# ThomasBrouwer/BNMTF

Hardware: AMD Instinct MI355X
Metric: Gibbs iterations/sec (BNMF, I=J=8192, K=64) (higher is better)
Workload: dtype f32

## Files before the change

bnmtf_amd/csrc/api.hip:

```cpp
#include <algorithm>
#include <atomic>
#include <chrono>
#include <cmath>
#include <cstdarg>
#include <cstdio>
#include <cstring>
#include <mutex>
#include <exception>
#include <new>
#include <system_error>
#include <thread>
#include <tuple>
#include <vector>

#include "model.h"
#include "comm.h"
#include "many.h"
#include "device_rng.h"

namespace bnmtf {

static thread_local char g_err[1024] = "";
void set_error(const char* fmt, ...) {
  va_list ap;
// ... 399 lines not shown
static bool build_handover(bnmtf_model* h, Dir& W, Dir& Rd) {
  if (!W.f_row_blk || !Rd.f_row_blk || W.f_npairs == 0 || Rd.f_npairs == 0) return false;
  const int nbW = (W.f_npairs + W.ho_ppb - 1) / W.ho_ppb, nbR = (Rd.f_npairs + Rd.ho_ppb - 1) / Rd.ho_ppb;
  if (nbR > 8192) return false;
  const size_t rowsW = W.f_slots, rowsR = Rd.f_slots;
  DevBuf<uint32_t> inv, dst_slot, dst_rank, count, sbase, stotal, rbase, rdata, rsize, limits;
  if (inv.alloc(std::max<size_t>(Rd.nslots, 1)) || dst_slot.alloc(std::max<size_t>(rowsW, 1) * 64) || dst_rank.alloc(std::max<size_t>(rowsW, 1) * 64) ||
      count.alloc((size_t)nbW * nbR) || sbase.alloc((size_t)nbW * nbR) || stotal.alloc(nbW) || rbase.alloc((size_t)nbW * nbR) || rdata.alloc(nbR) ||
      rsize.alloc(nbR) || limits.alloc(4, true)) return false;
  uint16_t *t_out = nullptr, *t_in = nullptr;
  if (dalloc(&t_out, ((rowsW + 1) / 2) * 128, true) || dalloc(&t_in, ((rowsR + 1) / 2) * 128, true)) return false;
  W.ho_out = reinterpret_cast<uint32_t*>(t_out); Rd.ho_in = reinterpret_cast<uint32_t*>(t_in);
  if (dalloc(&W.ho_pk, (size_t)nbW * nbR * 3, false) || dalloc(&Rd.ho_region_ofs, (size_t)nbR + 1, false)) return false;
  HandoverArgs a;
  a.w_off = W.f_off; a.w_pB = W.f_pair_base; a.w_pE = W.f_pair_E; a.w_umap = W.f_unit_map; a.w_npairs = W.f_npairs; a.w_ppb = W.ho_ppb; a.w_nb = nbW; a.w_inner = (uint32_t)Rd.nglob;
  a.r_off = Rd.f_off; a.r_pB = Rd.f_pair_base; a.r_pE = Rd.f_pair_E; a.r_umap = Rd.f_unit_map; a.r_npairs = Rd.f_npairs; a.r_ppb = Rd.ho_ppb; a.r_nb = nbR; a.r_inner = (uint32_t)W.nglob;
  a.r_row_blk = Rd.f_row_blk; a.r_ptr = Rd.slot_ptr; a.r_idx = Rd.idx;
  a.inv = inv.p; a.dst_slot = dst_slot.p; a.dst_rank = dst_rank.p; a.count = count.p;
  a.sbase = sbase.p; a.stotal = stotal.p; a.rbase = rbase.p; a.rdata = rdata.p; a.rsize = rsize.p;
  a.rofs = Rd.ho_region_ofs; a.t_out = t_out; a.t_in = t_in; a.pk = W.ho_pk; a.limits = limits.p;
  launch_handover_build(a, h->stream);
  uint32_t lim[4];
  if (hipMemcpyAsync(lim, limits.p, sizeof(lim), hipMemcpyDeviceToHost, h->stream) != hipSuccess || hipStreamSynchronize(h->stream) != hipSuccess) return false;
  const uint32_t lds_w = (W.ho_ppb == 8 ? 80u : 160u) * 1024u / 4u - (uint32_t)(W.KP * W.KP) - 256u;
  const uint32_t lds_r = (Rd.ho_ppb == 8 ? 80u : 160u) * 1024u / 4u - (uint32_t)(W.KP * W.KP) - 256u;
  if (lim[2] != 0 || lim[0] + 256u + 32u > lds_w || lim[0] + 32u > 65536u || lim[1] > lds_r || lim[1] > 65536u) return false;
  W.ho_lds_floats = std::max(W.ho_lds_floats, (int)lim[0] + 256 + 32);
  Rd.ho_lds_floats = std::max(Rd.ho_lds_floats, (int)lim[1]);
  if (dalloc(&Rd.ho_region, (size_t)lim[3] + 256) != BNMTF_OK) return false;
  Rd.ho_blocks = nbR;
  return true;
}

static int alloc_factor(Dir& d, int other_inner_pad) {
  d.xrows = std::max(d.nglob + 1, other_inner_pad);
  d.ldT = round_up(round_up(d.nglob, 32) + 32, 256);
  CHK(dalloc(&d.X, (size_t)d.xrows * d.KP));
  CHK(dalloc(&d.XT, (size_t)d.KP * d.ldT));
  CHK(dalloc(&d.XT2, (size_t)d.KP * d.ldT));
  const int nb = post_blocks(d.nglob);
  CHK(dalloc(&d.Cpart, (size_t)nb * d.KP * d.KP));
  CHK(dalloc(&d.spart, (size_t)nb * d.KP));
  CHK(dalloc(&d.s2part, (size_t)nb * d.KP));
  return BNMTF_OK;
}

static void free_dir(Dir& d) {
  dfree(d.big); dfree(d.slabs); dfree(d.lambda); dfree(d.slot_ptr); dfree(d.idx); dfree(d.q);
  dfree(d.X); dfree(d.XT); dfree(d.C64); dfree(d.C32);
  if (!d.gram_packed) { dfree(d.colsum); dfree(d.colsum2); }
  if (d.ev_sweep) (void)hipEventDestroy(d.ev_sweep);
  if (d.ev_gram) (void)hipEventDestroy(d.ev_gram);
  if (d.ev_gathered) (void)hipEventDestroy(d.ev_gathered);
  if (d.ev_gram_all) (void)hipEventDestroy(d.ev_gram_all);
  dfree(d.XT2); dfree(d.Cpart); dfree(d.spart); dfree(d.s2part); dfree(d.f_unit_map); dfree(d.f_pair_E);
  dfree(d.f_pair_base); dfree(d.f_off); dfree(d.f_off16); dfree(d.stats); dfree(d.f_gen_units);
  dfree(d.u_unit_map); dfree(d.u_pair_E); dfree(d.u_pair_base); dfree(d.u_off16);
  dfree(d.vb_stats);
  dfree(d.ho_in); dfree(d.ho_out); dfree(d.ho_pk); dfree(d.ho_region_ofs); dfree(d.ho_region); dfree(d.f_row_blk);
  dfree(d.mu); dfree(d.tauq); dfree(d.var); dfree(d.S2); dfree(d.S2T); dfree(d.XS); dfree(d.vb_asq); dfree(d.vb_vsq); dfree(d.mbits); dfree(d.XB); dfree(d.mslabs); dfree(d.xb_umax); dfree(d.xb_cexp); dfree(d.xb_mpart); dfree(d.numer); dfree(d.taup);
}

struct ScopedKernelTimer {
  bnmtf_model* h; int id; hipEvent_t a = nullptr, b = nullptr;
  bool on;
  ScopedKernelTimer(bnmtf_model* h_, int id_) : h(h_), id(id_), on(((h_->profiling >> id_) & 1u) && h_->iteration % h_->profile_stride == 0) {
    if (!on) return;
    auto get = [&]() {
      hipEvent_t e;
      if (!h->event_pool.empty()) { e = h->event_pool.back(); h->event_pool.pop_back(); }
      else (void)hipEventCreate(&e);
      return e;
    };
    a = get(); b = get();
    (void)hipEventRecord(a, h->stream);
  }
  ~ScopedKernelTimer() {
    if (!on) return;
    (void)hipEventRecord(b, h->stream);
    h->pending_events.push_back({id, {a, b}});
  }
};
static void drain_events(bnmtf_model* h) {
  for (auto& pe : h->pending_events) {
    float ms = 0.f;
    if (hipEventElapsedTime(&ms, pe.second.first, pe.second.second) == hipSuccess) {
      h->kernel_ms[pe.first] += ms;
      h->kernel_launches[pe.first] += 1;
    }
    h->event_pool.push_back(pe.second.first);
    h->event_pool.push_back(pe.second.second);
  }
  h->pending_events.clear();
}

struct HandoverScope {
  bnmtf_model* h;
  explicit HandoverScope(bnmtf_model* h_) : h(h_) {
    h->ho_active = h->ho_enabled && !h->comm && h->use_fast && !h->block_mode;
    if (!h->ho_active || !h->ho_regions_current) h->rows.ho_filled = h->cols.ho_filled = false;
    h->ho_regions_current = false;
  }
  void commit() { h->ho_regions_current = h->ho_active && h->rows.ho_filled; }
  ~HandoverScope() { h->ho_active = false; }
};
static void enqueue_gemm(bnmtf_model* h, Dir& d, const Dir& other, int kid, int part = 0);
static void enqueue_gemm(bnmtf_model* h, Dir& d, const Dir& other, int kid, int part) {
  GemmArgs g;
  g.big = d.big; g.ld = d.n_pad; g.X = other.X; g.slabs = d.slabs;
  g.n_pad = d.n_pad; g.split = d.split; g.inner_per_wave = d.ipw; g.tw = d.gemm_tw;
  const int rows_per_slice = 4 * d.ipw;
  const int s0 = (other.n0 + rows_per_slice - 1) / rows_per_slice, s1 = std::min(d.split, (other.n0 + other.n) / rows_per_slice);
  const bool have_local = h->comm && s1 > s0;
  if (part == 1) {
    if (!have_local) return;
    ScopedKernelTimer t(h, kid);
    g.split0 = s0; g.nsplit = s1 - s0;
    launch_gemm(g, d.KP, h->stream);
    return;
  }
  ScopedKernelTimer t(h, kid);
  if (part == 2 && have_local) {
    if (s0 > 0) { g.split0 = 0; g.nsplit = s0; launch_gemm(g, d.KP, h->stream); }
    if (s1 < d.split) { g.split0 = s1; g.nsplit = d.split - s1; launch_gemm(g, d.KP, h->stream); }
    return;
  }
  launch_gemm(g, d.KP, h->stream);
}
static bool vb_chip_ok(const Dir& d, const Dir& o) {
  if (!(d.mbits && o.XB && d.mslabs && d.nch == 1 && sweep_fast_supported(d.KP, d.pw))) return false;
  if (d.vb_path != 0) return d.vb_path == 1;
  return d.KP == 64 && d.use_wide;
}
static void enqueue_post(bnmtf_model* h, Dir& d, bool vb = false) {
  PostArgs g;
  memset(&g, 0, sizeof(g));
  g.X = d.X; g.rows = d.nglob; g.KP = d.KP; g.XT = d.XT; g.ldT = d.ldT; g.XT2 = d.XT2; g.ld2 = d.ldT;
  g.Cpart = d.Cpart; g.spart = d.spart; g.C64 = d.C64; g.C32 = d.C32; g.colsum = d.colsum;
  if (vb) { g.S2 = d.S2; g.S2T = d.S2T; g.s2part = d.s2part; g.colsum2 = d.colsum2; g.XS = d.XS; }
  if (vb && vb_chip_ok(h->rows, h->cols) && vb_chip_ok(h->cols, h->rows)) {
    g.XS = nullptr;
    g.mpart = d.xb_mpart; g.umax = d.xb_umax;
    d.xb_umax_posted = d.xb_mpart != nullptr;
  } else d.xb_umax_posted = false;
  g.snap = d.snap_dst; g.snapW = d.W; d.snap_dst = nullptr;
  launch_post(g, h->stream);
}
static int exchange_factor(bnmtf_model* h, Dir& d, Dir* next = nullptr, int next_kid = 0) {
  if (!h->comm) { enqueue_post(h, d); return BNMTF_OK; }
  const char* xe = getenv("BNMTF_EXCHANGE");
  if (xe && !strcmp(xe, "serial")) {
    PostArgs g;
    memset(&g, 0, sizeof(g));
    g.X = d.X; g.rows = d.nglob; g.KP = d.KP; g.XT = d.XT; g.ldT = d.ldT; g.XT2 = d.XT2; g.ld2 = d.ldT;
    g.Cpart = d.Cpart; g.spart = d.spart; g.C64 = d.C64; g.C32 = d.C32; g.colsum = d.colsum;
    launch_post_gram_rows(g, d.n0, d.n0 + d.n, h->stream);
    CHK(comm_allgather_factor(h->comm, d.X, d.KP, d.nglob, h->world, h->stream));
    CHK(comm_allreduce_sum(h->comm, d.C64, 64 * 64 + 64, h->stream));
    launch_gram_cast(d.C64, d.C32, d.KP * d.KP, h->stream);
    g.snap = d.snap_dst; g.snapW = d.W; d.snap_dst = nullptr;
    launch_post_layout(g, h->stream);
    d.gram_pending = false;
    return BNMTF_OK;
  }
  if (!h->xchg_stream) HIPCHK(hipStreamCreateWithFlags(&h->xchg_stream, hipStreamNonBlocking));
  for (hipEvent_t* e : {&d.ev_sweep, &d.ev_gram, &d.ev_gathered, &d.ev_gram_all})
    if (!*e) HIPCHK(hipEventCreateWithFlags(e, hipEventDisableTiming));
  PostArgs g;
  memset(&g, 0, sizeof(g));
  g.X = d.X; g.rows = d.nglob; g.KP = d.KP; g.XT = d.XT; g.ldT = d.ldT; g.XT2 = d.XT2; g.ld2 = d.ldT;
  g.Cpart = d.Cpart; g.spart = d.spart; g.C64 = d.C64; g.C32 = d.C32; g.colsum = d.colsum;
  HIPCHK(hipEventRecord(d.ev_sweep, h->stream));
  launch_post_gram_rows(g, d.n0, d.n0 + d.n, h->stream);
  HIPCHK(hipEventRecord(d.ev_gram, h->stream));
  if (next) enqueue_gemm(h, *next, d, next_kid, 1);
  HIPCHK(hipStreamWaitEvent(h->xchg_stream, d.ev_sweep, 0));
  CHK(comm_allgather_factor(h->comm, d.X, d.KP, d.nglob, h->world, h->xchg_stream));
  HIPCHK(hipEventRecord(d.ev_gathered, h->xchg_stream));
  HIPCHK(hipStreamWaitEvent(h->xchg_stream, d.ev_gram, 0));
  CHK(comm_allreduce_sum(h->comm, d.C64, 64 * 64 + 64, h->xchg_stream));
  launch_gram_cast(d.C64, d.C32, d.KP * d.KP, h->xchg_stream);
  HIPCHK(hipEventRecord(d.ev_gram_all, h->xchg_stream));
// ... 33 lines not shown
    s2.acc = nullptr;
    if (h->ho_active) { d.ho_filled = false; }
    launch_sweep_unit(s2, f, h->stream);
    h->last_sweep_fast = true;
    return;
  }
  if (h->use_fast && d.fast_ok && s.cond_k < 0 && s.mode != kSweepVB && (d.nch == 2 || sweep_fast_supported(d.KP, d.pw))) {
    FastArgs f;
    f.unit_map = d.f_unit_map; f.pair_E = d.f_pair_E; f.pair_base = d.f_pair_base; f.off = d.f_off;
    f.npairs = d.f_npairs; f.mz = d.mz; f.pw = d.nch == 2 ? d.pw_chunk : d.pw; f.nw = d.f_nw;
    f.nch = d.nch; f.mh = d.mh; f.pw1 = d.pw1; f.twin = d.use_twin ? 1 : 0;
    f.XoT = other.XT; f.ldT_o = other.ldT; f.XoT2 = other.XT2; f.ld2_o = other.ldT; f.Xo = other.X; f.Xo_rows = other.nglob;
    f.stats = want_stats ? d.stats : nullptr;
    SweepArgs s2 = s;
    s2.acc = nullptr;
    f.off16 = d.pair_ok ? d.f_off16 : nullptr;
    set_handover(h, d, other, f, !d.use_turns && d.nch == 1 && d.f_nw == d.ho_ppb && s.mode != kSweepVB);
#ifdef BNMTF_EXPERIMENTS
    if (d.use_wide && d.use_turns) launch_sweep_turns(s2, f, h->stream);
    else
#endif
    if (d.use_wide && !d.use_twin) launch_sweep_wide(s2, f, h->stream);
    else launch_sweep_fast(s2, f, h->stream);
    h->last_sweep_fast = true;
    if (d.f_gen_count == 0) return;
    s.unit_list = d.f_gen_units;
    s.n = d.f_gen_count;
  }
  launch_sweep(s, h->stream);
}
static SweepArgs sweep_args(bnmtf_model* h, Dir& d, const Dir& other, int mode, uint32_t stream_id) {
  SweepArgs s;
  memset(&s, 0, sizeof(s));
  s.min_x = mode == kSweepMode ? h->cur_min_x : 0.f;
  s.n = d.n; s.n0 = d.n0; s.K = d.W; s.KP = d.KP; s.mode = mode; s.cond_k = -1; s.qinit_only = 0; s.only_k = -1; s.vb_moments = 1; s.vb_stats = nullptr;
  s.col0 = h->col0;
  s.slabs = d.slabs; s.split = d.split; s.n_pad = d.n_pad; s.lambda = d.lambda;
  s.Xself = d.X; s.XselfT = nullptr; s.ldT_self = d.ldT;
  s.XoT = other.XT; s.ldT_o = other.ldT; s.C32 = other.C32;
  s.slot_ptr = d.slot_ptr; s.idx = d.idx; s.q = d.q;
  s.tau = h->tau_f;
  s.key0 = (uint32_t)h->seed; s.key1 = (uint32_t)(h->seed >> 32); s.it = (uint32_t)h->iteration; s.stream = stream_id;
  s.acc = nullptr;
  s.numer_out = d.numer; s.tau_out = d.taup;
  s.mu_self = d.mu; s.tau_self = d.tauq; s.var_self = d.var; s.S2self = d.S2; s.S2selfT = d.S2T;
  s.S2oT = other.S2T; s.colsum2_o = other.colsum2;
  return s;
}

static int upload_factor(bnmtf_model* h, Dir& d, const double* src) {
  std::vector<float> tmp((size_t)d.nglob * d.KP, 0.0f);
  for (int r = 0; r < d.nglob; ++r)
    for (int k = 0; k < d.W; ++k) tmp[(size_t)r * d.KP + k] = (float)src[(size_t)r * d.W + k];
  HIPCHK(hipMemcpyAsync(d.X, tmp.data(), tmp.size() * sizeof(float), hipMemcpyHostToDevice, h->stream));
  HIPCHK(hipStreamSynchronize(h->stream));
  enqueue_post(h, d);
  return BNMTF_OK;
}
static int download_matrix(bnmtf_model* h, const float* dev, int rows, int W, int KP, double* dst) {
  std::vector<float> tmp((size_t)rows * KP);
  HIPCHK(hipMemcpyAsync(tmp.data(), dev, tmp.size() * sizeof(float), hipMemcpyDeviceToHost, h->stream));
  HIPCHK(hipStreamSynchronize(h->stream));
  for (int r = 0; r < rows; ++r)
    for (int k = 0; k < W; ++k) dst[(size_t)r * W + k] = (double)tmp[(size_t)r * KP + k];
  return BNMTF_OK;
}
// ... 284 lines not shown
  if (hipMemcpyAsync(h->Rfull, R, (size_t)I * J * sizeof(float), hipMemcpyHostToDevice, h->stream) != hipSuccess) { set_error("copy R failed"); return fail(BNMTF_EHIP); }
  if (hipMemcpyAsync(h->Mtrain, M, (size_t)I * J, hipMemcpyHostToDevice, h->stream) != hipSuccess) { set_error("copy M failed"); return fail(BNMTF_EHIP); }
  if (h->small) {
    if (hipStreamSynchronize(h->stream) != hipSuccess) { set_error("bnmtf_create: uploads failed"); return fail(BNMTF_EHIP); }
    h->std_built = false;
    laps.lap("small-model arena");
  } else {
    if ((rcode = build_standard(h, p->lambda_S, p->comm_id))) return fail(rcode);
  }
  h->create_ms = std::chrono::duration<double, std::milli>(std::chrono::steady_clock::now() - t_create0).count();
  describe_model(h);
  *out = h;
  return BNMTF_OK;
} BNMTF_ABI_GUARD
}

namespace bnmtf {
static int build_standard(bnmtf_model* h, const double* lambda_S, const uint8_t* comm_id) {
  const auto t_create0 = std::chrono::steady_clock::now();
  const int I = h->I, J = h->J;
  const int Wr = h->K, Wc = h->L > 0 ? h->L : h->K;
  struct { int K, L, rank, world; const uint8_t* comm_id; const double* lambda_S; uint64_t seed; } pv{h->K, h->L, h->rank, h->world, comm_id, lambda_S, h->seed};
  auto* p = &pv;
  auto fail = [&](int rc) { return rc; };
  CreateLaps laps;
  int rcode;
  const std::vector<uint32_t> rc = h->rows.obs_count, cc = h->cols.obs_count;
  rcode = build_dir(h->rows, I, J, Wr, p->rank, p->world, h->lam_rows.data(), h->Rfull, h->Mtrain, I, J, true, rc, h->stream);
  if (rcode) return fail(rcode);
  rcode = build_dir(h->cols, J, I, Wc, p->rank, p->world, h->lam_cols.data(), h->Rfull, h->Mtrain, I, J, false, cc, h->stream);
  if (rcode) return fail(rcode);
  laps.lap("both directions built (total)");
  h->rows.obs_count = rc; h->cols.obs_count = cc;
  if ((rcode = alloc_factor(h->rows, h->cols.inner_pad))) return fail(rcode);
  if ((rcode = alloc_factor(h->cols, h->rows.inner_pad))) return fail(rcode);

  laps.lap("factor buffers");
  if (!h->Ad && (rcode = dalloc(&h->Ad, (size_t)I * 64))) return fail(rcode);
  if (!h->Bd && (rcode = dalloc(&h->Bd, (size_t)J * 64))) return fail(rcode);
  if (p->L > 0 && (rcode = dalloc(&h->S, (size_t)p->K * p->L))) return fail(rcode);
  if (p->L > 0 && (rcode = bnmtf_alloc_extras(h, p->lambda_S))) return fail(rcode);

  if (p->world > 1) {
    if ((rcode = comm_create(&h->comm, p->comm_id, p->rank, p->world, h->stream))) return fail(rcode);
    const double mine[4] = {(double)(uint32_t)p->seed, (double)(uint32_t)(p->seed >> 32), -(double)(uint32_t)p->seed, -(double)(uint32_t)(p->seed >> 32)};
    double got[4];
    if (hipMemcpy(h->acc, mine, sizeof(mine), hipMemcpyHostToDevice) != hipSuccess) { set_error("seed check: copy failed"); return fail(BNMTF_EHIP); }
    if ((rcode = comm_allreduce_max(h->comm, h->acc, 4, h->stream))) return fail(rcode);
    if (hipStreamSynchronize(h->stream) != hipSuccess || hipMemcpy(got, h->acc, sizeof(got), hipMemcpyDeviceToHost) != hipSuccess) { set_error("seed check: copy failed"); return fail(BNMTF_EHIP); }
    (void)hipMemset(h->acc, 0, 4 * sizeof(double));
    if (memcmp(mine, got, sizeof(mine)) != 0) {
      set_error("bnmtf_create: the ranks were given different seeds (this rank %llu): a sharded model needs one shared seed", (unsigned long long)p->seed);
      return fail(BNMTF_EINVAL);
    }
  } else if (getenv("BNMTF_FORCE_COMM")) {
    uint8_t id[128];
    if ((rcode = comm_unique_id(id))) return fail(rcode);
    if ((rcode = comm_create(&h->comm, id, 0, 1, h->stream))) return fail(rcode);
  }

  {
    const char* e = getenv("BNMTF_HANDOVER");
    auto blocks = [](const Dir& d) { return d.ho_ppb > 0 ? d.f_npairs / d.ho_ppb : 0; };
    const bool want = p->L == 0 && !h->comm && (e ? atoi(e) != 0 : std::min(blocks(h->rows), blocks(h->cols)) >= 64);
    const auto t_ho0 = std::chrono::steady_clock::now();
    if (want && build_handover(h, h->rows, h->cols) && build_handover(h, h->cols, h->rows)) h->rows.ho_ready = h->cols.ho_ready = h->ho_enabled = true;
    if (const char* r = getenv("BNMTF_HANDOVER_REFRESH")) h->ho_refresh = (uint64_t)std::max(1, atoi(r));
    if (const char* u = getenv("BNMTF_UNIT")) h->uw_force = atoi(u) == 1;
// ... 556 lines not shown
```

bnmtf_amd/csrc/kernel_gemm.hip:

```cpp
#include <cstdlib>
#include <cstring>

#include "kernels.h"
#include "many.h"

namespace bnmtf {

typedef float f32x16 __attribute__((ext_vector_type(16)));
typedef float f32x4 __attribute__((ext_vector_type(4)));

template <int MT, int U, int WPS>
__global__ __launch_bounds__(256, WPS) void gemm_kernel(GemmArgs a) {
  constexpr int KP = MT * 32;
  constexpr int NACC = MT * 4 * 16;
  __shared__ float red[2][NACC * 64];

  const int lane = threadIdx.x & 63, wave = threadIdx.x >> 6;
  const int h = lane >> 5, c = lane & 31;
  const int col0 = blockIdx.x * 128;
  const int s = blockIdx.y + a.split0;
  const int ipw = a.inner_per_wave;
  const size_t r0 = (size_t)(s * 4 + wave) * ipw + h;

  const float* bp = a.big + r0 * (size_t)a.ld + col0 + 4 * c;
  const float* xp = a.X + r0 * KP + c;
  const size_t bstep = 2 * (size_t)a.ld;

  f32x16 acc[MT][4];
#pragma unroll
  for (int mt = 0; mt < MT; ++mt)
#pragma unroll
    for (int t = 0; t < 4; ++t)
#pragma unroll
      for (int g = 0; g < 16; ++g) acc[mt][t][g] = 0.0f;

// ... 54 lines not shown
      for (int t = 0; t < 4; ++t)
#pragma unroll
        for (int g = 0; g < 16; ++g) dst[((mt * 4 + t) * 16 + g) * 64 + lane] = acc[mt][t][g];
  };
  auto add = [&](const float* src) {
#pragma unroll
    for (int mt = 0; mt < MT; ++mt)
#pragma unroll
      for (int t = 0; t < 4; ++t)
#pragma unroll
        for (int g = 0; g < 16; ++g) acc[mt][t][g] += src[((mt * 4 + t) * 16 + g) * 64 + lane];
  };
  if (wave >= 2) put(red[wave - 2]);
  __syncthreads();
  if (wave < 2) add(red[wave]);
  __syncthreads();
  if (wave == 1) put(red[0]);
  __syncthreads();
  if (wave == 0) {
    add(red[0]);
    float* out = a.slabs + ((size_t)s * a.n_pad + col0) * KP;
#pragma unroll
    for (int mt = 0; mt < MT; ++mt)
#pragma unroll
      for (int t = 0; t < 4; ++t)
#pragma unroll
        for (int g4 = 0; g4 < 4; ++g4) {
          f32x4 v = {acc[mt][t][4 * g4], acc[mt][t][4 * g4 + 1], acc[mt][t][4 * g4 + 2], acc[mt][t][4 * g4 + 3]};
          *reinterpret_cast<f32x4*>(out + (size_t)(4 * c + t) * KP + mt * 32 + 8 * g4 + 4 * h) = v;
        }
  }
}

typedef __bf16 bf16x8 __attribute__((ext_vector_type(8)));
typedef uint32_t u32x4 __attribute__((ext_vector_type(4)));
typedef float f32x2g __attribute__((ext_vector_type(2)));

typedef __bf16 bf16x2 __attribute__((ext_vector_type(2)));
typedef float f32x2c __attribute__((ext_vector_type(2)));
__device__ __forceinline__ uint32_t pack_rne(float a0, float a1) {
  f32x2c v; v.x = a0; v.y = a1;
  return __builtin_bit_cast(uint32_t, __builtin_convertvector(v, bf16x2));
}
__device__ __forceinline__ void split3(const float (&v)[8], u32x4& hi, u32x4& mid, u32x4& lo) {
#pragma unroll
  for (int p = 0; p < 4; ++p) {
    const float a0 = v[2 * p], a1 = v[2 * p + 1];
    const uint32_t h = pack_rne(a0, a1);
    hi[p] = h;
    const float b0 = a0 - __builtin_bit_cast(float, h << 16);
    const float b1 = a1 - __builtin_bit_cast(float, h & 0xffff0000u);
    const uint32_t m = pack_rne(b0, b1);
    mid[p] = m;
    const float c0 = b0 - __builtin_bit_cast(float, m << 16);
    const float c1 = b1 - __builtin_bit_cast(float, m & 0xffff0000u);
    lo[p] = pack_rne(c0, c1);
  }
}

template <int MT, int NSET, int TW, int RB = 1>
__device__ __forceinline__ void gemm_bf16x3_body(const GemmArgs& a) {
  typedef float f32xT __attribute__((ext_vector_type(TW)));
  constexpr int KP = MT * 32;
  constexpr int NACC = MT * TW * 16;
  __shared__ float red[2][NACC * 64];

  const int lane = threadIdx.x & 63, wave = threadIdx.x >> 6;
  const int h = lane >> 5, c = lane & 31;
  const int col0 = blockIdx.x * (32 * TW);
  const int s = blockIdx.y + a.split0;
  const int ipw = a.inner_per_wave;
  const size_t r0 = (size_t)(s * 4 + wave) * ipw + 8 * h;

  const float* bp = a.big + r0 * (size_t)a.ld + col0 + TW * c;
  const float* xp = a.X + r0 * KP + c;

  f32x16 acc[MT][TW];
#pragma unroll
  for (int mt = 0; mt < MT; ++mt)
#pragma unroll
    for (int t = 0; t < TW; ++t)
#pragma unroll
      for (int g = 0; g < 16; ++g) acc[mt][t][g] = 0.0f;

  f32xT braw[NSET][8];
  float araw[NSET][MT][8];
  auto load_step = [&](int gi, f32xT (&b)[8], float (&av)[MT][8]) {
    const float* bpg = bp + (size_t)gi * 16 * (size_t)a.ld;
    const float* xpg = xp + (size_t)gi * 16 * KP;
#pragma unroll
    for (int rr = 0; rr < 8; ++rr) {
      b[rr] = __builtin_nontemporal_load(reinterpret_cast<const f32xT*>(bpg + (size_t)rr * a.ld));
#pragma unroll
      for (int mt = 0; mt < MT; ++mt) av[mt][rr] = xpg[rr * KP + mt * 32];
    }
  };
  auto mul_step = [&](const f32xT (&b)[8], const float (&av)[MT][8]) {
    u32x4 ah[MT], am[MT], al[MT];
#pragma unroll
    for (int mt = 0; mt < MT; ++mt) split3(av[mt], ah[mt], am[mt], al[mt]);
#pragma unroll
    for (int t = 0; t < TW; ++t) {
      float bv[8];
#pragma unroll
      for (int rr = 0; rr < 8; ++rr) bv[rr] = b[rr][t];
      u32x4 bh, bm, bl;
      split3(bv, bh, bm, bl);
#pragma unroll
      for (int mt = 0; mt < MT; ++mt) {
        f32x16 d = acc[mt][t];
        d = __builtin_amdgcn_mfma_f32_32x32x16_bf16(__builtin_bit_cast(bf16x8, al[mt]), __builtin_bit_cast(bf16x8, bh), d, 0, 0, 0);
        d = __builtin_amdgcn_mfma_f32_32x32x16_bf16(__builtin_bit_cast(bf16x8, ah[mt]), __builtin_bit_cast(bf16x8, bl), d, 0, 0, 0);
        d = __builtin_amdgcn_mfma_f32_32x32x16_bf16(__builtin_bit_cast(bf16x8, am[mt]), __builtin_bit_cast(bf16x8, bm), d, 0, 0, 0);
        d = __builtin_amdgcn_mfma_f32_32x32x16_bf16(__builtin_bit_cast(bf16x8, am[mt]), __builtin_bit_cast(bf16x8, bh), d, 0, 0, 0);
        d = __builtin_amdgcn_mfma_f32_32x32x16_bf16(__builtin_bit_cast(bf16x8, ah[mt]), __builtin_bit_cast(bf16x8, bm), d, 0, 0, 0);
        d = __builtin_amdgcn_mfma_f32_32x32x16_bf16(__builtin_bit_cast(bf16x8, ah[mt]), __builtin_bit_cast(bf16x8, bh), d, 0, 0, 0);
        acc[mt][t] = d;
      }
#ifdef BNMTF_GEMM_SLEEP
      __builtin_amdgcn_s_sleep(BNMTF_GEMM_SLEEP);
#endif
    }
  };
#ifdef BNMTF_GEMM_STAGGER
  for (int i = 0; i < wave; ++i) __builtin_amdgcn_s_sleep(BNMTF_GEMM_STAGGER);
#endif
  const int nsteps = ipw / 16;
  const int last = nsteps - 1;
  if constexpr (RB == 0) {
    int nl = 0;
#pragma unroll
    for (int j = 0; j < NSET - 1; ++j)
      if (j < nsteps) load_step(nl++, braw[j], araw[j]);
// ... 32 lines not shown
      for (int t = 0; t < TW; ++t)
#pragma unroll
        for (int g = 0; g < 16; ++g) dst[((mt * TW + t) * 16 + g) * 64 + lane] = acc[mt][t][g];
  };
  auto add = [&](const float* src) {
#pragma unroll
    for (int mt = 0; mt < MT; ++mt)
#pragma unroll
      for (int t = 0; t < TW; ++t)
#pragma unroll
        for (int g = 0; g < 16; ++g) acc[mt][t][g] += src[((mt * TW + t) * 16 + g) * 64 + lane];
  };
  if (wave >= 2) put(red[wave - 2]);
  __syncthreads();
  if (wave < 2) add(red[wave]);
  __syncthreads();
  if (wave == 1) put(red[0]);
  __syncthreads();
  if (wave == 0) {
    add(red[0]);
    float* out = a.slabs + ((size_t)s * a.n_pad + col0) * KP;
#pragma unroll
    for (int mt = 0; mt < MT; ++mt)
#pragma unroll
      for (int t = 0; t < TW; ++t)
#pragma unroll
        for (int g4 = 0; g4 < 4; ++g4) {
          f32x4 v = {acc[mt][t][4 * g4], acc[mt][t][4 * g4 + 1], acc[mt][t][4 * g4 + 2], acc[mt][t][4 * g4 + 3]};
          *reinterpret_cast<f32x4*>(out + (size_t)(TW * c + t) * KP + mt * 32 + 8 * g4 + 4 * h) = v;
        }
  }
}

template <int MT, int NSET, int TW, int RB = 1>
__global__ __launch_bounds__(256, (TW == 4 ? 1 : 2)) void gemm_bf16x3_kernel(GemmArgs a) { gemm_bf16x3_body<MT, NSET, TW, RB>(a); }
template <int MT, int NSET, int TW>
__global__ __launch_bounds__(256, (TW == 4 ? 1 : 2)) void gemm_bf16x3_many(const GemmArgs* list, int) { gemm_bf16x3_body<MT, NSET, TW, 1>(load_pack(list, blockIdx.z)); }

#ifndef BNMTF_GEMM_NSET
#define BNMTF_GEMM_NSET 3
#endif
void launch_gemm(const GemmArgs& a, int KP, hipStream_t st) {
  const int ns = a.nsplit > 0 ? a.nsplit : a.split;
  if (ns <= 0) return;
  dim3 grid(a.n_pad / 128, ns), block(256);
#ifdef BNMTF_EXPERIMENTS
  const char* mode = getenv("BNMTF_GEMM");
  const bool f32 = mode && !strcmp(mode, "f32");
#else
  constexpr bool f32 = false;
#endif
  if (!f32) {
#ifdef BNMTF_EXPERIMENTS
    const char* ring = getenv("BNMTF_GEMM_RING");
    if (ring && !strcmp(ring, "old")) {
      if (KP == 32) hipLaunchKernelGGL((gemm_bf16x3_kernel<1, 3, 4, 0>), grid, block, 0, st, a);
      else if (a.tw == 2) hipLaunchKernelGGL((gemm_bf16x3_kernel<2, 3, 2, 0>), dim3(a.n_pad / 64, ns), block, 0, st, a);
      else          hipLaunchKernelGGL((gemm_bf16x3_kernel<2, 3, 4, 0>), grid, block, 0, st, a);
      return;
    }
#endif
    if (g_recorder) {
      if (KP == 32) record_launch((const void*)gemm_bf16x3_many<1, BNMTF_GEMM_NSET, 4>, grid, block, 0, a);
      else if (a.tw == 2) record_launch((const void*)gemm_bf16x3_many<2, BNMTF_GEMM_NSET, 2>, dim3(a.n_pad / 64, ns), block, 0, a);
      else record_launch((const void*)gemm_bf16x3_many<2, BNMTF_GEMM_NSET, 4>, grid, block, 0, a);
      return;
    }
    if (KP == 32) hipLaunchKernelGGL((gemm_bf16x3_kernel<1, BNMTF_GEMM_NSET, 4>), grid, block, 0, st, a);
    else if (a.tw == 2) hipLaunchKernelGGL((gemm_bf16x3_kernel<2, BNMTF_GEMM_NSET, 2>), dim3(a.n_pad / 64, ns), block, 0, st, a);
    else          hipLaunchKernelGGL((gemm_bf16x3_kernel<2, BNMTF_GEMM_NSET, 4>), grid, block, 0, st, a);
    return;
  }
#ifdef BNMTF_EXPERIMENTS
  if (KP == 32) hipLaunchKernelGGL((gemm_kernel<1, 16, 2>), grid, block, 0, st, a);
  else          hipLaunchKernelGGL((gemm_kernel<2, 16, 1>), grid, block, 0, st, a);
#endif
}

}
```

bnmtf_amd/csrc/kernel_post.hip:

```cpp
#include "kernels.h"
#include "many.h"

namespace bnmtf {

__device__ __forceinline__ void tri_tile(int p, int NT, int* ty, int* tx) {
  int y = 0, rem = p;
  while (rem >= NT - y) { rem -= NT - y; ++y; }
  *ty = y; *tx = y + rem;
}

template <bool VB>
__device__ __forceinline__ void post_body(const PostArgs& a) {
  constexpr int RB = kPostRows;
  constexpr int LD = 68, LDD = 66;
  __shared__ double smem[(RB * LDD * sizeof(double) >= (VB ? 2 : 1) * RB * LD * sizeof(float) ? RB * LDD : ((VB ? 2 : 1) * RB * LD + 1) / 2) + 4 * 64];
  float* tile0 = reinterpret_cast<float*>(smem);
  float* tile1 = tile0 + RB * LD;
  double* dtile = smem;
  double* dred = smem + RB * LDD;
  const int KP = a.KP, tid = threadIdx.x;
  const int r0 = (a.blk0 + blockIdx.x) * RB;
  const int nr = min(RB, a.rows - r0);
  const bool do_layout = a.do_layout && (!a.do_gram || blockIdx.y == 0), do_gram = a.do_gram && (!a.do_layout || blockIdx.y == 1);
  if (do_gram) {
    for (int pass = 0; pass < (VB ? 2 : 1); ++pass) {
      const float* src = pass == 0 ? a.X : a.S2;
      if (pass == 1) __syncthreads();
      for (int t = tid; t < RB * KP; t += 256) {
        const int r = t / KP, k = t % KP;
        dtile[r * LDD + k] = (r < nr && (a.do_layout || (r0 + r >= a.own0 && r0 + r < a.own1))) ? (double)src[(size_t)(r0 + r) * KP + k] : 0.0;
      }
      __syncthreads();
// ... 37 lines not shown
          __syncthreads();
          dred[grp * 64 + col] = mx;
          __syncthreads();
          if (tid < KP) {
            const float m = (float)fmax(fmax(dred[tid], dred[64 + tid]), fmax(dred[128 + tid], dred[192 + tid]));
            a.mpart[(size_t)blockIdx.x * 2 * KP + (pass == 0 ? KP : 0) + tid] = pass == 0 ? m * m : m;
          }
        }
      }
    }
    return;
  }
  if (!do_layout) return;
  const float* src = a.X;
  for (int pass = 0; pass < (VB ? 2 : 1); ++pass) {
    float* tile = pass == 0 ? tile0 : tile1;
    if (pass == 1) src = a.S2;
    for (int t = tid; t < RB * KP; t += 256) {
      const int r = t / KP, k = t % KP;
      tile[r * LD + k] = r < nr ? src[(size_t)(r0 + r) * KP + k] : 0.f;
    }
    __syncthreads();
    float* T1 = pass == 0 ? a.XT : a.S2T;
    if (T1)
      for (int t = tid; t < RB * KP; t += 256) {
        const int k = t / RB, r = t % RB;
        if (r < nr) T1[(size_t)k * a.ldT + r0 + r] = tile[r * LD + k];
      }
    if (pass == 0 && a.snap)
      for (int t = tid; t < RB * a.snapW; t += 256) {
        const int r = t / a.snapW, k = t % a.snapW;
        if (r < nr) a.snap[(size_t)(r0 + r) * a.snapW + k] = tile[r * LD + k];
      }
    if (pass == 0 && a.XT2)
      for (int t = tid; t < RB * KP; t += 256) {
        const int kp = t / (2 * RB), rem = t % (2 * RB), r = rem >> 1, c = rem & 1;
        if (r < nr) a.XT2[((size_t)kp * a.ld2 + r0 + r) * 2 + c] = tile[r * LD + 2 * kp + c];
      }
    if (pass == 1 && a.XS)
      for (int t = tid; t < RB * KP; t += 256) {
        const int k = t / RB, r = t % RB;
        if (r < nr) *reinterpret_cast<float2*>(a.XS + ((size_t)k * a.ldT + r0 + r) * 2) = float2{tile0[r * LD + k], tile1[r * LD + k]};
      }
  }
}
template <bool VB>
__global__ __launch_bounds__(256) void post_kernel(PostArgs a) { post_body<VB>(a); }
template <bool VB>
__global__ __launch_bounds__(256) void post_many(const PostArgs* list, int) { post_body<VB>(load_pack(list, blockIdx.z)); }

__device__ __forceinline__ void gram_reduce_body(const PostArgs& a, int nblk) {
  __shared__ double red[1024];
  const int KP = a.KP;
  if (a.S2 && a.mpart && a.umax && (int)blockIdx.x == (int)gridDim.x - 2) {
    float* fred = reinterpret_cast<float*>(red);
    const int c = threadIdx.x & 127, g8 = threadIdx.x >> 7;
    float m = 0.f;
    if (c < 2 * KP)
      for (int b0 = g8; b0 < nblk; b0 += 8 * 8) {
        float w[8];
#pragma unroll
        for (int u = 0; u < 8; ++u) w[u] = b0 + 8 * u < nblk ? a.mpart[(size_t)(b0 + 8 * u) * 2 * KP + c] : 0.f;
#pragma unroll
        for (int u = 0; u < 8; ++u) m = fmaxf(m, w[u]);
      }
    fred[threadIdx.x] = m;
// ... 112 lines not shown
```

bnmtf_amd/csrc/kernels.h:

```cpp
#pragma once
#include <hip/hip_runtime.h>
#include <stdint.h>

namespace bnmtf {

constexpr uint32_t kStreamRows = 0, kStreamCols = 1, kStreamS = 2, kStreamTau = 3, kStreamHook = 8;

struct GemmArgs {
  const float* big; int ld;
  const float* X;
  float* slabs;
  int n_pad, split, inner_per_wave;
  int tw;
  int split0 = 0, nsplit = 0;
};
void launch_gemm(const GemmArgs& a, int KP, hipStream_t st);

struct MaskGemmArgs {
  const uint32_t* bits; int ldw;
  const uint32_t* XB; int rows_pad; const int* cexp;
  float* slabs;
  int n_pad, split, inner_per_wave;
  int ncol = 0;
};
void launch_maskgemm(const MaskGemmArgs& a, int KP, hipStream_t st);
void launch_vb_planes(const float* S2, const float* E, int rows, int rows_pad, int KP, unsigned* umax, bool have_max, int* cexp, uint32_t* XB, hipStream_t st);
void launch_mask_bits(const uint8_t* M, int I, int J, int by_rows, int unit0, int n, int m, int n_pad, int ldw, uint32_t* bits, hipStream_t st);

struct GramArgs {
  const float* X; const float* S2; int rows, KP;
  double* C64; float* C32; double* colsum; double* colsum2;
};
void launch_gram(const GramArgs& a, hipStream_t st);

enum SweepMode { kSweepDraw = 0, kSweepMode = 1, kSweepVB = 2 };

struct SweepArgs {
  int n, n0;
  const int* unit_list;
  int K, KP;
  int mode;
  int cond_k;
  int qinit_only;
  int only_k;
  uint32_t col0;
  float min_x;
  int vb_moments;
// ... 44 lines not shown
bool sweep_fast_supported(int KP, int pw);
bool sweep_two_chunks_plan(int KP, int m, int* mh, int* pw, int* pw1);
void launch_sweep_fast(const SweepArgs& a, const FastArgs& f, hipStream_t st);
void launch_sweep_small(const SweepArgs& a, const FastArgs& f, hipStream_t st);
constexpr int kUnitMaxUnits = 2048;
constexpr int kUnitMaxSlots = 32;
bool sweep_unit_supported(int KP, int pw);
void launch_sweep_unit(const SweepArgs& a, const FastArgs& f, hipStream_t st);
constexpr int kWideMaxSlots = 32;
constexpr int kTwinPanelStride = 8448;
bool sweep_wide_supported(int KP, int pw);
void launch_sweep_wide(const SweepArgs& a, const FastArgs& f, hipStream_t st);
bool sweep_turns_supported(int KP, int pw);
void launch_sweep_turns(const SweepArgs& a, const FastArgs& f, hipStream_t st);
bool sweep_vb_supported(int KP, int pw);
bool sweep_vb_cov_supported(int KP, int pw);
int sweep_vb_blocks(int npairs, int nw = 8);
void launch_sweep_vb(const SweepArgs& a, const FastArgs& f, hipStream_t st);
void launch_vb_pieces(int n, int n0, int KP, int K, const float* mu, const float* tauq, const float* ex, const float* var,
                      const float* lambda, const float* asq, const float* vsq, double* out, hipStream_t st);
void launch_vb_pieces_slabs(int n, int n0, int KP, int K, const float* mu, const float* tauq, const float* ex, const float* var,
                            const float* lambda, const float* mslabs, int msplit, int n_pad, double* out, hipStream_t st);

struct PostArgs {
  const float* X; int rows, KP;
  float* XT; int ldT; float* XT2; int ld2;
  double* Cpart; double* spart;
  double* C64; float* C32; double* colsum;
  const float* S2; float* S2T; double* s2part; double* colsum2;
  float* XS;
  float* mpart; unsigned* umax;
  int do_layout, do_gram, blk0, own0, own1;
  float* snap; int snapW;
};
void launch_post(const PostArgs& a, hipStream_t st);
void launch_post_layout(const PostArgs& a, hipStream_t st);
void launch_post_gram_rows(const PostArgs& a, int own0, int own1, hipStream_t st);
void launch_masked_operand(const float* R, const uint8_t* M, int I, int J, int by_rows, int unit0, int n, int m, float* out, int ld, hipStream_t st);
constexpr int kMaxOtherBlocks = 4;
struct ResidualSpec { int n; const float* A[kMaxOtherBlocks]; const float* B[kMaxOtherBlocks]; int KP[kMaxOtherBlocks]; int W[kMaxOtherBlocks]; };
void launch_residual_operand(const float* R, const uint8_t* M, int I, int J, int by_rows, int unit0, int n, int m, float* out, int ld,
                             const ResidualSpec& rs, hipStream_t st);
void launch_missing_lists(const uint8_t* M, int I, int J, int by_rows, int unit0, int n, int m, const uint32_t* ptr, uint32_t* idx, hipStream_t st);
struct HandoverArgs {
  const uint32_t* w_off; const uint32_t* w_pB; const uint32_t* w_pE; const int* w_umap; int w_npairs, w_ppb, w_nb; uint32_t w_inner;
  const uint32_t* r_off; const uint32_t* r_pB; const uint32_t* r_pE; const int* r_umap; int r_npairs, r_ppb, r_nb; uint32_t r_inner;
  const uint16_t* r_row_blk;
  const uint32_t* r_ptr; const uint32_t* r_idx;
  uint32_t* inv; uint32_t* dst_slot; uint32_t* dst_rank; uint32_t* count;
  uint32_t* sbase; uint32_t* stotal; uint32_t* rbase; uint32_t* rdata; uint32_t* rsize;
  uint32_t* rofs; uint16_t* t_out; uint16_t* t_in; uint32_t* pk;
  uint32_t* limits;
};
void launch_handover_build(const HandoverArgs& a, hipStream_t st);
void launch_gram_cast(const double* C64, float* C32, int n, hipStream_t st);
constexpr int kPostRows = 32;
inline int post_blocks(int rows) { return (rows + kPostRows - 1) / kPostRows; }

struct FinishArgs {
  const double* Cr64; const double* Cc64; const double* sr; const double* sc; int KP;
  const double* acc;
  const double* stats; int nstats;
  double n_obs, sumR, sumR2;
  double alpha, beta;
  int update;
  uint32_t key0, key1, it;
// ... 245 lines not shown
```

bnmtf_amd/csrc/model.h:

```cpp
#pragma once
#include <hip/hip_runtime.h>
#include <stdint.h>

#include <string>
#include <vector>

#include "../../include/bnmtf_hip.h"
#include "kernels.h"

namespace bnmtf {

void set_error(const char* fmt, ...);

#define HIPCHK(expr)                                                                          \
  do {                                                                                        \
    hipError_t e_ = (expr);                                                                   \
    if (e_ != hipSuccess) {                                                                   \
      ::bnmtf::set_error("%s failed: %s (%s:%d)", #expr, hipGetErrorString(e_), __FILE__, __LINE__); \
      return BNMTF_EHIP;                                                                      \
    }                                                                                         \
  } while (0)

#define CHK(expr)                  \
  do {                             \
    int rc_ = (expr);              \
    if (rc_ != BNMTF_OK) return rc_; \
  } while (0)

struct Dir {
  int nglob = 0;
  int n = 0, n0 = 0;
  int m = 0;
  int W = 0, KP = 0;
  int n_pad = 0, split = 1, ipw = 0, inner_pad = 0;
  float* big = nullptr;
  float* slabs = nullptr;
  float* lambda = nullptr;
  uint32_t* slot_ptr = nullptr;
  uint32_t* idx = nullptr;
  float* q = nullptr;
  size_t nslots = 0, nmiss = 0;
  float* X = nullptr;  int xrows = 0;
  float* XT = nullptr; int ldT = 0;
  float* XT2 = nullptr;
  double* Cpart = nullptr; double* spart = nullptr; double* s2part = nullptr;
  int* f_unit_map = nullptr; uint32_t* f_pair_E = nullptr; uint32_t* f_pair_base = nullptr; uint32_t* f_off = nullptr;
  int f_npairs = 0, f_emax = 0, mz = 0; size_t f_slots = 0;
  int f_nw = 8;
  uint32_t* f_off16 = nullptr; bool pair_ok = false;
  int pw = 0;
  int nch = 1, mh = 0, pw_chunk = 0, pw1 = 0;
  int* f_gen_units = nullptr; int f_gen_count = 0;
  bool uw_ok = false; int u_nw = 4, u_emax = 0;
  int* u_unit_map = nullptr; uint32_t* u_pair_E = nullptr; uint32_t* u_pair_base = nullptr; uint32_t* u_off16 = nullptr;
  double* stats = nullptr; int stats_blocks = 0;
  bool fast_ok = false;
  int gemm_tw = 4;
  bool use_turns = false;
  bool use_wide = false;
  int vb_path = 0;
  double* C64 = nullptr; float* C32 = nullptr; double* colsum = nullptr;
  uint32_t* ho_in = nullptr;
  uint32_t* ho_out = nullptr;
  uint32_t* ho_pk = nullptr;
  uint32_t* ho_region_ofs = nullptr;
  float* ho_region = nullptr;
  int ho_blocks = 0, ho_lds_floats = 0;
  bool ho_ready = false;
  mutable bool ho_filled = false;
  uint16_t* f_row_blk = nullptr;
  int ho_ppb = 0;
  bool use_twin = false;
  bool gram_packed = false;
  hipEvent_t ev_sweep = nullptr, ev_gram = nullptr, ev_gathered = nullptr, ev_gram_all = nullptr;
  float* snap_dst = nullptr;
  bool gram_pending = false;
  bool gemm_ahead = false;
// ... 102 lines not shown
```

Before: 2514.

## Presplit factor matrix into bf16x3 MFMA fragments during post pass

```diff
diff --git a/bnmtf_amd/csrc/api.hip b/bnmtf_amd/csrc/api.hip
--- a/bnmtf_amd/csrc/api.hip
+++ b/bnmtf_amd/csrc/api.hip
@@ -455,12 +455,14 @@
   return true;
 }
 
-static int alloc_factor(Dir& d, int other_inner_pad) {
+static int alloc_factor(Dir& d, int other_inner_pad, bool presplit = false) {
   d.xrows = std::max(d.nglob + 1, other_inner_pad);
   d.ldT = round_up(round_up(d.nglob, 32) + 32, 256);
   CHK(dalloc(&d.X, (size_t)d.xrows * d.KP));
   CHK(dalloc(&d.XT, (size_t)d.KP * d.ldT));
   CHK(dalloc(&d.XT2, (size_t)d.KP * d.ldT));
+  d.xs_valid = false;
+  if (presplit) CHK(dalloc(&d.Xs, (size_t)round_up(d.xrows, 32) * d.KP * 3 / 2));
   const int nb = post_blocks(d.nglob);
   CHK(dalloc(&d.Cpart, (size_t)nb * d.KP * d.KP));
   CHK(dalloc(&d.spart, (size_t)nb * d.KP));
@@ -470,7 +472,7 @@
 
 static void free_dir(Dir& d) {
   dfree(d.big); dfree(d.slabs); dfree(d.lambda); dfree(d.slot_ptr); dfree(d.idx); dfree(d.q);
-  dfree(d.X); dfree(d.XT); dfree(d.C64); dfree(d.C32);
+  dfree(d.X); dfree(d.XT); dfree(d.Xs); dfree(d.C64); dfree(d.C32);
   if (!d.gram_packed) { dfree(d.colsum); dfree(d.colsum2); }
   if (d.ev_sweep) (void)hipEventDestroy(d.ev_sweep);
   if (d.ev_gram) (void)hipEventDestroy(d.ev_gram);
@@ -532,6 +534,7 @@
   GemmArgs g;
   g.big = d.big; g.ld = d.n_pad; g.X = other.X; g.slabs = d.slabs;
   g.n_pad = d.n_pad; g.split = d.split; g.inner_per_wave = d.ipw; g.tw = d.gemm_tw;
+  g.Xs = !h->comm && other.xs_valid ? other.Xs : nullptr;
   const int rows_per_slice = 4 * d.ipw;
   const int s0 = (other.n0 + rows_per_slice - 1) / rows_per_slice, s1 = std::min(d.split, (other.n0 + other.n) / rows_per_slice);
   const bool have_local = h->comm && s1 > s0;
@@ -567,10 +570,12 @@
     d.xb_umax_posted = d.xb_mpart != nullptr;
   } else d.xb_umax_posted = false;
   g.snap = d.snap_dst; g.snapW = d.W; d.snap_dst = nullptr;
+  g.Xs = d.Xs; d.xs_valid = d.Xs != nullptr;
   launch_post(g, h->stream);
 }
 static int exchange_factor(bnmtf_model* h, Dir& d, Dir* next = nullptr, int next_kid = 0) {
   if (!h->comm) { enqueue_post(h, d); return BNMTF_OK; }
+  d.xs_valid = false;
   const char* xe = getenv("BNMTF_EXCHANGE");
   if (xe && !strcmp(xe, "serial")) {
     PostArgs g;
@@ -670,6 +675,7 @@
 static SweepArgs sweep_args(bnmtf_model* h, Dir& d, const Dir& other, int mode, uint32_t stream_id) {
   SweepArgs s;
   memset(&s, 0, sizeof(s));
+  d.xs_valid = false;
   s.min_x = mode == kSweepMode ? h->cur_min_x : 0.f;
   s.n = d.n; s.n0 = d.n0; s.K = d.W; s.KP = d.KP; s.mode = mode; s.cond_k = -1; s.qinit_only = 0; s.only_k = -1; s.vb_moments = 1; s.vb_stats = nullptr;
   s.col0 = h->col0;
@@ -1020,8 +1026,10 @@
   if (rcode) return fail(rcode);
   laps.lap("both directions built (total)");
   h->rows.obs_count = rc; h->cols.obs_count = cc;
-  if ((rcode = alloc_factor(h->rows, h->cols.inner_pad))) return fail(rcode);
-  if ((rcode = alloc_factor(h->cols, h->rows.inner_pad))) return fail(rcode);
+  const char* ps_env = getenv("BNMTF_GEMM_PRESPLIT");
+  const bool presplit = h->L == 0 && p->world == 1 && !(ps_env && atoi(ps_env) == 0);
+  if ((rcode = alloc_factor(h->rows, h->cols.inner_pad, presplit))) return fail(rcode);
+  if ((rcode = alloc_factor(h->cols, h->rows.inner_pad, presplit))) return fail(rcode);
 
   laps.lap("factor buffers");
   if (!h->Ad && (rcode = dalloc(&h->Ad, (size_t)I * 64))) return fail(rcode);
diff --git a/bnmtf_amd/csrc/bf16x3.h b/bnmtf_amd/csrc/bf16x3.h
--- /dev/null
+++ b/bnmtf_amd/csrc/bf16x3.h
@@ -0,0 +1,37 @@
+#pragma once
+#include <hip/hip_runtime.h>
+
+#include <cstdint>
+
+namespace bnmtf {
+
+typedef __bf16 bf16x8 __attribute__((ext_vector_type(8)));
+typedef uint32_t u32x4 __attribute__((ext_vector_type(4)));
+
+typedef __bf16 bf16x2 __attribute__((ext_vector_type(2)));
+typedef float f32x2c __attribute__((ext_vector_type(2)));
+__device__ __forceinline__ uint32_t pack_rne(float a0, float a1) {
+  f32x2c v; v.x = a0; v.y = a1;
+  return __builtin_bit_cast(uint32_t, __builtin_convertvector(v, bf16x2));
+}
+__device__ __forceinline__ void split3(const float (&v)[8], u32x4& hi, u32x4& mid, u32x4& lo) {
+#pragma unroll
+  for (int p = 0; p < 4; ++p) {
+    const float a0 = v[2 * p], a1 = v[2 * p + 1];
+    const uint32_t h = pack_rne(a0, a1);
+    hi[p] = h;
+    const float b0 = a0 - __builtin_bit_cast(float, h << 16);
+    const float b1 = a1 - __builtin_bit_cast(float, h & 0xffff0000u);
+    const uint32_t m = pack_rne(b0, b1);
+    mid[p] = m;
+    const float c0 = b0 - __builtin_bit_cast(float, m << 16);
+    const float c1 = b1 - __builtin_bit_cast(float, m & 0xffff0000u);
+    lo[p] = pack_rne(c0, c1);
+  }
+}
+
+__host__ __device__ inline size_t xs_index(size_t rb, int term, int mt, int MT, int lane) {
+  return ((rb * 3 + term) * MT + mt) * 64 + lane;
+}
+
+}
diff --git a/bnmtf_amd/csrc/kernel_gemm.hip b/bnmtf_amd/csrc/kernel_gemm.hip
--- a/bnmtf_amd/csrc/kernel_gemm.hip
+++ b/bnmtf_amd/csrc/kernel_gemm.hip
@@ -1,6 +1,9 @@
 #include <cstdlib>
 #include <cstring>
 
+#include <type_traits>
+
+#include "bf16x3.h"
 #include "kernels.h"
 #include "many.h"
 
@@ -121,33 +124,7 @@
   }
 }
 
-typedef __bf16 bf16x8 __attribute__((ext_vector_type(8)));
-typedef uint32_t u32x4 __attribute__((ext_vector_type(4)));
-typedef float f32x2g __attribute__((ext_vector_type(2)));
-
-typedef __bf16 bf16x2 __attribute__((ext_vector_type(2)));
-typedef float f32x2c __attribute__((ext_vector_type(2)));
-__device__ __forceinline__ uint32_t pack_rne(float a0, float a1) {
-  f32x2c v; v.x = a0; v.y = a1;
-  return __builtin_bit_cast(uint32_t, __builtin_convertvector(v, bf16x2));
-}
-__device__ __forceinline__ void split3(const float (&v)[8], u32x4& hi, u32x4& mid, u32x4& lo) {
-#pragma unroll
-  for (int p = 0; p < 4; ++p) {
-    const float a0 = v[2 * p], a1 = v[2 * p + 1];
-    const uint32_t h = pack_rne(a0, a1);
-    hi[p] = h;
-    const float b0 = a0 - __builtin_bit_cast(float, h << 16);
-    const float b1 = a1 - __builtin_bit_cast(float, h & 0xffff0000u);
-    const uint32_t m = pack_rne(b0, b1);
-    mid[p] = m;
-    const float c0 = b0 - __builtin_bit_cast(float, m << 16);
-    const float c1 = b1 - __builtin_bit_cast(float, m & 0xffff0000u);
-    lo[p] = pack_rne(c0, c1);
-  }
-}
-
-template <int MT, int NSET, int TW, int RB = 1>
+template <int MT, int NSET, int TW, int RB = 1, bool PS = false>
 __device__ __forceinline__ void gemm_bf16x3_body(const GemmArgs& a) {
   typedef float f32xT __attribute__((ext_vector_type(TW)));
   constexpr int KP = MT * 32;
@@ -163,6 +140,7 @@
 
   const float* bp = a.big + r0 * (size_t)a.ld + col0 + TW * c;
   const float* xp = a.X + r0 * KP + c;
+  const u32x4* xsp = PS ? reinterpret_cast<const u32x4*>(a.Xs) + xs_index((size_t)(s * 4 + wave) * ipw / 16, 0, 0, MT, lane) : nullptr;
 
   f32x16 acc[MT][TW];
 #pragma unroll
@@ -172,22 +150,35 @@
 #pragma unroll
       for (int g = 0; g < 16; ++g) acc[mt][t][g] = 0.0f;
 
+  typedef typename std::conditional<PS, u32x4[MT][3], float[MT][8]>::type AStep;
   f32xT braw[NSET][8];
-  float araw[NSET][MT][8];
-  auto load_step = [&](int gi, f32xT (&b)[8], float (&av)[MT][8]) {
+  AStep araw[NSET];
+  auto load_step = [&](int gi, f32xT (&b)[8], AStep& av) {
     const float* bpg = bp + (size_t)gi * 16 * (size_t)a.ld;
-    const float* xpg = xp + (size_t)gi * 16 * KP;
-#pragma unroll
-    for (int rr = 0; rr < 8; ++rr) {
+#pragma unroll
+    for (int rr = 0; rr < 8; ++rr)
       b[rr] = __builtin_nontemporal_load(reinterpret_cast<const f32xT*>(bpg + (size_t)rr * a.ld));
-#pragma unroll
-      for (int mt = 0; mt < MT; ++mt) av[mt][rr] = xpg[rr * KP + mt * 32];
-    }
-  };
-  auto mul_step = [&](const f32xT (&b)[8], const float (&av)[MT][8]) {
+    if constexpr (PS) {
+      const u32x4* xg = xsp + (size_t)gi * 3 * MT * 64;
+#pragma unroll
+      for (int term = 0; term < 3; ++term)
+#pragma unroll
+        for (int mt = 0; mt < MT; ++mt) av[mt][term] = xg[(term * MT + mt) * 64];
+    } else {
+      const float* xpg = xp + (size_t)gi * 16 * KP;
+#pragma unroll
+      for (int rr = 0; rr < 8; ++rr)
+#pragma unroll
+        for (int mt = 0; mt < MT; ++mt) av[mt][rr] = xpg[rr * KP + mt * 32];
+    }
+  };
+  auto mul_step = [&](const f32xT (&b)[8], const AStep& av) {
     u32x4 ah[MT], am[MT], al[MT];
 #pragma unroll
-    for (int mt = 0; mt < MT; ++mt) split3(av[mt], ah[mt], am[mt], al[mt]);
+    for (int mt = 0; mt < MT; ++mt) {
+      if constexpr (PS) { ah[mt] = av[mt][0]; am[mt] = av[mt][1]; al[mt] = av[mt][2]; }
+      else split3(av[mt], ah[mt], am[mt], al[mt]);
+    }
 #pragma unroll
     for (int t = 0; t < TW; ++t) {
       float bv[8];
@@ -286,14 +277,22 @@
   }
 }
 
-template <int MT, int NSET, int TW, int RB = 1>
-__global__ __launch_bounds__(256, (TW == 4 ? 1 : 2)) void gemm_bf16x3_kernel(GemmArgs a) { gemm_bf16x3_body<MT, NSET, TW, RB>(a); }
+template <int MT, int NSET, int TW, int RB = 1, bool PS = false>
+__global__ __launch_bounds__(256, (TW == 4 ? 1 : 2)) void gemm_bf16x3_kernel(GemmArgs a) { gemm_bf16x3_body<MT, NSET, TW, RB, PS>(a); }
 template <int MT, int NSET, int TW>
 __global__ __launch_bounds__(256, (TW == 4 ? 1 : 2)) void gemm_bf16x3_many(const GemmArgs* list, int) { gemm_bf16x3_body<MT, NSET, TW, 1>(load_pack(list, blockIdx.z)); }
 
 #ifndef BNMTF_GEMM_NSET
 #define BNMTF_GEMM_NSET 3
 #endif
+template <int MT, int TW>
+constexpr int presplit_sets() { return MT == 2 && TW == 4 ? 4 : BNMTF_GEMM_NSET; }
+template <int MT, int TW>
+static void launch_bf16x3(const GemmArgs& a, int ns, hipStream_t st) {
+  const dim3 grid(a.n_pad / (32 * TW), ns), block(256);
+  if (a.Xs) hipLaunchKernelGGL((gemm_bf16x3_kernel<MT, presplit_sets<MT, TW>(), TW, 1, true>), grid, block, 0, st, a);
+  else      hipLaunchKernelGGL((gemm_bf16x3_kernel<MT, BNMTF_GEMM_NSET, TW, 1, false>), grid, block, 0, st, a);
+}
 void launch_gemm(const GemmArgs& a, int KP, hipStream_t st) {
   const int ns = a.nsplit > 0 ? a.nsplit : a.split;
   if (ns <= 0) return;
@@ -320,9 +319,9 @@
       else record_launch((const void*)gemm_bf16x3_many<2, BNMTF_GEMM_NSET, 4>, grid, block, 0, a);
       return;
     }
-    if (KP == 32) hipLaunchKernelGGL((gemm_bf16x3_kernel<1, BNMTF_GEMM_NSET, 4>), grid, block, 0, st, a);
-    else if (a.tw == 2) hipLaunchKernelGGL((gemm_bf16x3_kernel<2, BNMTF_GEMM_NSET, 2>), dim3(a.n_pad / 64, ns), block, 0, st, a);
-    else          hipLaunchKernelGGL((gemm_bf16x3_kernel<2, BNMTF_GEMM_NSET, 4>), grid, block, 0, st, a);
+    if (KP == 32) launch_bf16x3<1, 4>(a, ns, st);
+    else if (a.tw == 2) launch_bf16x3<2, 2>(a, ns, st);
+    else launch_bf16x3<2, 4>(a, ns, st);
     return;
   }
 #ifdef BNMTF_EXPERIMENTS
diff --git a/bnmtf_amd/csrc/kernel_post.hip b/bnmtf_amd/csrc/kernel_post.hip
--- a/bnmtf_amd/csrc/kernel_post.hip
+++ b/bnmtf_amd/csrc/kernel_post.hip
@@ -1,3 +1,4 @@
+#include "bf16x3.h"
 #include "kernels.h"
 #include "many.h"
 
@@ -101,6 +102,23 @@
         const int r = t / a.snapW, k = t % a.snapW;
         if (r < nr) a.snap[(size_t)(r0 + r) * a.snapW + k] = tile[r * LD + k];
       }
+    if (pass == 0 && a.Xs) {
+      const int MT = KP / 32;
+      u32x4* xs = reinterpret_cast<u32x4*>(a.Xs);
+      for (int t = tid; t < 2 * MT * 64; t += 256) {
+        const int lane = t & 63, mt = (t >> 6) % MT, j = (t >> 6) / MT;
+        const float* col = tile + (16 * j + 8 * (lane >> 5)) * LD + 32 * mt + (lane & 31);
+        float v[8];
+#pragma unroll
+        for (int rr = 0; rr < 8; ++rr) v[rr] = col[rr * LD];
+        u32x4 hi, mid, lo;
+        split3(v, hi, mid, lo);
+        const size_t rb = (size_t)(r0 / 16 + j);
+        xs[xs_index(rb, 0, mt, MT, lane)] = hi;
+        xs[xs_index(rb, 1, mt, MT, lane)] = mid;
+        xs[xs_index(rb, 2, mt, MT, lane)] = lo;
+      }
+    }
     if (pass == 0 && a.XT2)
       for (int t = tid; t < RB * KP; t += 256) {
         const int kp = t / (2 * RB), rem = t % (2 * RB), r = rem >> 1, c = rem & 1;
diff --git a/bnmtf_amd/csrc/kernels.h b/bnmtf_amd/csrc/kernels.h
--- a/bnmtf_amd/csrc/kernels.h
+++ b/bnmtf_amd/csrc/kernels.h
@@ -13,6 +13,7 @@
   int n_pad, split, inner_per_wave;
   int tw;
   int split0 = 0, nsplit = 0;
+  const uint32_t* Xs = nullptr;
 };
 void launch_gemm(const GemmArgs& a, int KP, hipStream_t st);
 
@@ -123,6 +124,7 @@
   float* mpart; unsigned* umax;
   int do_layout, do_gram, blk0, own0, own1;
   float* snap; int snapW;
+  uint32_t* Xs;
 };
 void launch_post(const PostArgs& a, hipStream_t st);
 void launch_post_layout(const PostArgs& a, hipStream_t st);
diff --git a/bnmtf_amd/csrc/model.h b/bnmtf_amd/csrc/model.h
--- a/bnmtf_amd/csrc/model.h
+++ b/bnmtf_amd/csrc/model.h
@@ -43,6 +43,7 @@
   float* X = nullptr;  int xrows = 0;
   float* XT = nullptr; int ldT = 0;
   float* XT2 = nullptr;
+  uint32_t* Xs = nullptr; bool xs_valid = false;
   double* Cpart = nullptr; double* spart = nullptr; double* s2part = nullptr;
   int* f_unit_map = nullptr; uint32_t* f_pair_E = nullptr; uint32_t* f_pair_base = nullptr; uint32_t* f_off = nullptr;
   int f_npairs = 0, f_emax = 0, mz = 0; size_t f_slots = 0;
```

After: 2529, median of 6. No clear change (+0.6%).
